# GATECH-EIC/BNS-GCN

Hardware: AMD Instinct MI355X
Metric: training throughput (full-graph edges/s), reddit-shaped graphsage 3-layer h=256, sampling-rate=0.1 (higher is better)
Workload: dtype fp32; 1 GPU; model=graphsage, dataset=reddit, n_layers=3, n_hidden=256, n_nodes=232965, n_edges=114756398, use_pp=True, partition=metis, parallelism=partition-parallel p1

## Files before the change

### bnsgcn_amd/ops/functional.py

```python
from __future__ import annotations

import torch
from torch.autograd import Function

from . import reference as ref
from ._ext import get_ext, use_hip



def _worklist_of(indptr):
    wl = getattr(indptr, "_bns_worklist", None)
    if wl is None:
        from .csr_torch import build_worklist
        wl = build_worklist(indptr)
        indptr._bns_worklist = wl
    return wl


def spmm_sum_raw(indptr, indices, x, src_scale=None, dst_scale=None, out=None):
    if use_hip(x):
        wrow, wbeg, wend, wave_start, zero_rows = _worklist_of(indptr)
        acc = out is not None
        if not acc:
            out = torch.empty(indptr.numel() - 1, x.shape[1],
# ... 180 lines not shown
                g_er = e.segment_sum_edges(*_worklist_of(indptr)[:4], None,
                                           grad, ctx.n_dst)
            return g_el, g_er, None, None, None, None, None, None
        if ctx.needs_input_grad[0]:
            g_el = torch.zeros(ctx.n_src, grad.shape[1], dtype=grad.dtype,
                               device=grad.device)
            g_el.index_add_(0, indices.long(), grad)
        if ctx.needs_input_grad[1]:
            g_er = torch.zeros(ctx.n_dst, grad.shape[1], dtype=grad.dtype,
                               device=grad.device)
            row = torch.repeat_interleave(
                torch.arange(ctx.n_dst, device=grad.device),
                indptr[1:] - indptr[:-1])
            g_er.index_add_(0, row, grad)
        return g_el, g_er, None, None, None, None, None, None


def sddmm_add(el, er, indptr, indices, indptr_t, indices_t, eperm_t,
              slope=None):
    return _SDDMMAdd.apply(el, er, indptr, indices, indptr_t, indices_t,
                           eperm_t, slope)


class _SegmentSoftmax(Function):
    @staticmethod
    def forward(ctx, logits, indptr):
        alpha = segment_softmax_raw(indptr, logits)
        ctx.save_for_backward(alpha, indptr)
        return alpha

    @staticmethod
    def backward(ctx, grad):
        alpha, indptr = ctx.saved_tensors
        return segment_softmax_bwd_raw(indptr, alpha, grad.contiguous()), None


def segment_softmax(logits, indptr):
    return _SegmentSoftmax.apply(logits, indptr)


import os as _os

_GEMM_MODE = _os.environ.get("BNSGCN_GEMM", "auto")


class _Linear(Function):

    @staticmethod
    def forward(ctx, x, weight, bias):
        ctx.save_for_backward(x, weight)
        ctx.has_bias = bias is not None
        if use_hip(x) and _GEMM_MODE == "hip":
            return get_ext().gemm_nt_bias(x, weight, bias)
        return torch.nn.functional.linear(x, weight, bias)

    @staticmethod
    def backward(ctx, grad):
        x, weight = ctx.saved_tensors
        grad = grad.contiguous()
        gx = gw = gb = None
        if use_hip(x):
            e = get_ext()
            if ctx.needs_input_grad[0]:
                gx = e.gemm_nn(grad, weight) if _GEMM_MODE == "hip" \
                    else grad @ weight
            if ctx.needs_input_grad[1]:
                gw = e.gemm_tn(grad, x)
            if ctx.has_bias and ctx.needs_input_grad[2]:
                return gx, gw, e.syncbn_stats(grad)[0]
        else:
            if ctx.needs_input_grad[0]:
                gx = grad @ weight
            if ctx.needs_input_grad[1]:
                gw = grad.t() @ x
        if ctx.has_bias and ctx.needs_input_grad[2]:
            gb = grad.sum(0)
        return gx, gw, gb


def linear(x, weight, bias=None):
    return _Linear.apply(x, weight, bias)


class _BiasAdd(Function):

    @staticmethod
    def forward(ctx, h, bias):
        return h + bias

    @staticmethod
    def backward(ctx, grad):
        gb = None
        if ctx.needs_input_grad[1]:
            gb = get_ext().syncbn_stats(grad.contiguous())[0] \
                if use_hip(grad) else grad.sum(0)
        return grad, gb


def bias_add(h, bias):
    return _BiasAdd.apply(h, bias)


class _LayerNormF(Function):

    @staticmethod
    def forward(ctx, x, weight, bias, eps, act):
        x = x.contiguous()
        y, mean, rstd = get_ext().ln_fwd(x, weight, bias, eps, int(act))
        ctx.save_for_backward(x, weight, bias, mean, rstd)
        ctx.act = int(act)
        return y

    @staticmethod
    def backward(ctx, dy):
        x, w, b, mean, rstd = ctx.saved_tensors
        dx, dw, db = get_ext().ln_bwd(x, dy.contiguous(), w, b, mean, rstd,
                                      ctx.act)
        return dx, dw, db, None, None


def layer_norm(x, weight, bias, eps: float = 1e-5, act: bool = False):
    if use_hip(x) and x.shape[-1] <= 1024 and x.dtype == torch.float32:
        return _LayerNormF.apply(x, weight, bias, eps, act)
    y = torch.nn.functional.layer_norm(x, (x.shape[-1],), weight, bias, eps)
    return torch.relu(y) if act else y


class _DropoutF(Function):

    @staticmethod
    def forward(ctx, x, keep, seed):
        ctx.keep, ctx.seed = keep, seed
        return get_ext().dropout_apply(x.contiguous(), keep, seed)

    @staticmethod
    def backward(ctx, dy):
        return (get_ext().dropout_apply(dy.contiguous(), ctx.keep, ctx.seed),
                None, None)


def dropout(x, p: float, training: bool):
    if not training or p <= 0.0:
        return x
    if use_hip(x) and x.dtype == torch.float32:
        seed = int(torch.randint(0, 2**62, (1,)).item())
        return _DropoutF.apply(x, 1.0 - p, seed)
    return torch.nn.functional.dropout(x, p, training)


def segment_softmax2_raw(indptr1, logits1, indptr2, logits2):
    if use_hip(logits1):
        return get_ext().segment_softmax2(indptr1, logits1, indptr2, logits2,
                                          1.0, 0)[:2]
    return ref.segment_softmax2(indptr1, logits1, indptr2, logits2)


def segment_softmax2_bwd_raw(indptr1, a1, g1, indptr2, a2, g2):
    if use_hip(a1):
        return get_ext().segment_softmax2_backward(indptr1, a1, g1,
                                                   indptr2, a2, g2, 1.0, 0)
    return ref.segment_softmax2_backward(indptr1, a1, g1, indptr2, a2, g2)


class _SegmentSoftmax2(Function):

    @staticmethod
# ... 67 lines not shown
```

### bnsgcn_amd/ops/hip/common.h

```cpp
#pragma once
#include <hip/hip_runtime.h>
#include <cstdint>

#define WAVE 64
#define DEV_INLINE __device__ __forceinline__

struct WorkList {
  const int32_t* __restrict__ row;
  const int64_t* __restrict__ beg;
  const int64_t* __restrict__ end;
  const int32_t* __restrict__ wave_start;
};

struct WaveItems { int lane, beg, end; };
struct WorkItem { int row; bool atomic; int64_t beg, end; };

DEV_INLINE int xcd_remap_block(int b, int nb) {
  const int q = nb / 8, r = nb % 8;
  const int xcd = b % 8, j = b / 8;
  return (xcd < r) ? xcd * (q + 1) + j : r * (q + 1) + (xcd - r) * q + j;
}

template <int SUBW>
DEV_INLINE WaveItems wave_items(const WorkList& wl) {
// ... 7 lines not shown
  const int row = wl.row[it];
  const bool atomic = row < 0;
  return {atomic ? ~row : row, atomic, wl.beg[it], wl.end[it]};
}

struct Chunk { int cid; float ssc; int nv; };

template <int SUBW>
DEV_INLINE Chunk load_chunk(const int32_t* __restrict__ indices,
                            const float* __restrict__ src_scale, int64_t e0,
                            int64_t end, int lane) {
  Chunk c = {0, 1.0f, (int)((end - e0 < SUBW) ? (end - e0) : SUBW)};
  if (lane < c.nv) {
    c.cid = indices[e0 + lane];
    if (src_scale) c.ssc = src_scale[c.cid];
  }
  return c;
}

DEV_INLINE void atomic_add(float* p, float v) { atomicAdd(p, v); }
DEV_INLINE void atomic_add(float2* p, float2 v) {
  float* f = reinterpret_cast<float*>(p);
  atomicAdd(f + 0, v.x); atomicAdd(f + 1, v.y);
}
DEV_INLINE void atomic_add(float4* p, float4 v) {
  float* f = reinterpret_cast<float*>(p);
  atomicAdd(f + 0, v.x); atomicAdd(f + 1, v.y);
  atomicAdd(f + 2, v.z); atomicAdd(f + 3, v.w);
}

template <bool ACC>
DEV_INLINE void store_row(float* dst, float v, bool atomic, float s = 1.0f) {
  if (atomic) atomic_add(dst, s * v);
  else if (ACC) *dst = fmaf(s, v, *dst);
  else *dst = s * v;
}
template <bool ACC>
DEV_INLINE void store_row(float2* dst, float2 v, bool atomic, float s = 1.0f) {
  if (atomic) {
    atomic_add(dst, make_float2(s * v.x, s * v.y));
  } else if (ACC) {
    const float2 pv = *dst;
    *dst = make_float2(fmaf(s, v.x, pv.x), fmaf(s, v.y, pv.y));
  } else {
    *dst = make_float2(s * v.x, s * v.y);
  }
}
template <bool ACC>
DEV_INLINE void store_row(float4* dst, float4 v, bool atomic, float s = 1.0f) {
  if (atomic) {
    atomic_add(dst, make_float4(s * v.x, s * v.y, s * v.z, s * v.w));
  } else if (ACC) {
    const float4 pv = *dst;
    *dst = make_float4(fmaf(s, v.x, pv.x), fmaf(s, v.y, pv.y),
                       fmaf(s, v.z, pv.z), fmaf(s, v.w, pv.w));
  } else {
    *dst = make_float4(s * v.x, s * v.y, s * v.z, s * v.w);
  }
}

DEV_INLINE uint32_t mulhi32(uint32_t a, uint32_t b) {
  return (uint32_t)(((uint64_t)a * b) >> 32);
}

struct P4 { uint32_t c0, c1, c2, c3; };

DEV_INLINE P4 philox4x32(uint32_t c0, uint32_t c1, uint32_t c2, uint32_t c3,
                         uint32_t k0, uint32_t k1) {
  const uint32_t M0 = 0xD2511F53u, M1 = 0xCD9E8D57u;
  const uint32_t W0 = 0x9E3779B9u, W1 = 0xBB67AE85u;
#pragma unroll
  for (int r = 0; r < 10; ++r) {
    uint32_t hi0 = mulhi32(c0, M0), lo0 = c0 * M0;
    uint32_t hi1 = mulhi32(c2, M1), lo1 = c2 * M1;
    uint32_t n0 = hi1 ^ c1 ^ k0;
    uint32_t n1 = lo1;
    uint32_t n2 = hi0 ^ c3 ^ k1;
    uint32_t n3 = lo0;
    c0 = n0; c1 = n1; c2 = n2; c3 = n3;
    k0 += W0; k1 += W1;
  }
  return {c0, c1, c2, c3};
}
```

### bnsgcn_amd/ops/hip/kernels.hip

```cpp
#include <hip/hip_runtime.h>
#include <torch/extension.h>
#include <ATen/cuda/CUDAContext.h>
#include <c10/util/Optional.h>
#include <algorithm>
#include "common.h"

namespace {


DEV_INLINE void f4_axpy(float4& a, float ss, const float4 v) {
  a.x += ss * v.x; a.y += ss * v.y; a.z += ss * v.z; a.w += ss * v.w;
}

template <bool ACC, int SUBW>
__global__ __launch_bounds__(256) void spmm_sum_vec4_kernel(
    const int32_t* __restrict__ wrow, const int64_t* __restrict__ wbeg,
    const int64_t* __restrict__ wend, const int32_t* __restrict__ wave_start,
    const int32_t* __restrict__ indices, const float* __restrict__ x,
    const float* __restrict__ src_scale, const float* __restrict__ dst_scale,
    float* __restrict__ out, int f4) {
  const WorkList wl = {wrow, wbeg, wend, wave_start};
  const WaveItems wi = wave_items<SUBW>(wl);
  const int lane = wi.lane;
  const float4* __restrict__ x4 = reinterpret_cast<const float4*>(x);
  float4* __restrict__ out4 = reinterpret_cast<float4*>(out);

  for (int it = wi.beg; it < wi.end; ++it) {
    const WorkItem wk = work_item(wl, it);
    const float ds = dst_scale ? dst_scale[wk.row] : 1.0f;
    for (int f0 = 0; f0 < f4; f0 += 2 * SUBW) {
      const int fA = f0 + lane;
      const int fB = fA + SUBW;
      const bool hasA = fA < f4, hasB = fB < f4;
      float4 acc0 = {0.f, 0.f, 0.f, 0.f}, acc1 = {0.f, 0.f, 0.f, 0.f};
      for (int64_t e0 = wk.beg; e0 < wk.end; e0 += SUBW) {
        const Chunk ch = load_chunk<SUBW>(indices, src_scale, e0, wk.end, lane);
#pragma unroll 4
        for (int k = 0; k < ch.nv; ++k) {
          const int c = __shfl(ch.cid, k, SUBW);
          const float ss = src_scale ? __shfl(ch.ssc, k, SUBW) : 1.0f;
          const int64_t base = (int64_t)c * f4;
          if (hasA) f4_axpy(acc0, ss, x4[base + fA]);
          if (hasB) f4_axpy(acc1, ss, x4[base + fB]);
        }
      }
      const int64_t ob = (int64_t)wk.row * f4;
      if (hasA) store_row<ACC>(&out4[ob + fA], acc0, wk.atomic, ds);
      if (hasB) store_row<ACC>(&out4[ob + fB], acc1, wk.atomic, ds);
    }
  }
}

template <bool ACC, int G>
__global__ __launch_bounds__(256) void spmm_sum_narrow_kernel(
    const int32_t* __restrict__ wrow, const int64_t* __restrict__ wbeg,
    const int64_t* __restrict__ wend, const int32_t* __restrict__ wave_start,
    const int32_t* __restrict__ indices, const float* __restrict__ x,
    const float* __restrict__ src_scale, const float* __restrict__ dst_scale,
    float* __restrict__ out, int f4) {
  constexpr int NG = WAVE / G;
  const WorkList wl = {wrow, wbeg, wend, wave_start};
  const WaveItems wi = wave_items<WAVE>(wl);
  const int lane = wi.lane;
  const int g = lane / G, j = lane % G;
  const bool has = j < f4;
  const float4* __restrict__ x4 = reinterpret_cast<const float4*>(x);
  float4* __restrict__ out4 = reinterpret_cast<float4*>(out);

  for (int it = wi.beg; it < wi.end; ++it) {
    const WorkItem wk = work_item(wl, it);
    const float ds = dst_scale ? dst_scale[wk.row] : 1.0f;
    float4 acc = {0.f, 0.f, 0.f, 0.f};
    for (int64_t e0 = wk.beg; e0 < wk.end; e0 += WAVE) {
      const Chunk ch = load_chunk<WAVE>(indices, src_scale, e0, wk.end, lane);
#pragma unroll 4
      for (int k = 0; k < ch.nv; k += NG) {
        const int kk = k + g;
        const int c = __shfl(ch.cid, kk, WAVE);
        const float ss = src_scale ? __shfl(ch.ssc, kk, WAVE) : 1.0f;
        if (has && kk < ch.nv) f4_axpy(acc, ss, x4[(int64_t)c * f4 + j]);
      }
    }
#pragma unroll
    for (int off = G; off < WAVE; off <<= 1) {
      acc.x += __shfl_xor(acc.x, off, WAVE);
      acc.y += __shfl_xor(acc.y, off, WAVE);
      acc.z += __shfl_xor(acc.z, off, WAVE);
      acc.w += __shfl_xor(acc.w, off, WAVE);
// ... 278 lines not shown
}


DEV_INLINE float wave_reduce_sum(float v) {
#pragma unroll
  for (int off = 32; off > 0; off >>= 1) v += __shfl_xor(v, off, WAVE);
  return v;
}

DEV_INLINE float wave_reduce_max(float v) {
#pragma unroll
  for (int off = 32; off > 0; off >>= 1) v = fmaxf(v, __shfl_xor(v, off, WAVE));
  return v;
}

__global__ __launch_bounds__(256) void sddmm_add_kernel(
    const int32_t* __restrict__ wrow, const int64_t* __restrict__ wbeg,
    const int64_t* __restrict__ wend, const int32_t* __restrict__ wave_start,
    const int32_t* __restrict__ indices, const float* __restrict__ el,
    const float* __restrict__ er, float* __restrict__ out, int H,
    float slope) {
  const WorkList wl = {wrow, wbeg, wend, wave_start};
  const WaveItems wi = wave_items<WAVE>(wl);
  for (int it = wi.beg; it < wi.end; ++it) {
    const WorkItem wk = work_item(wl, it);
    for (int64_t e0 = wk.beg; e0 < wk.end; e0 += WAVE) {
      const int64_t e = e0 + wi.lane;
      if (e >= wk.end) break;
      const int64_t c = indices[e];
      for (int h = 0; h < H; ++h) {
        float v = el[c * H + h] + er[(int64_t)wk.row * H + h];
        if (slope >= 0.f && v < 0.f) v *= slope;
        out[e * H + h] = v;
      }
    }
  }
}

__global__ void segment_softmax_kernel(const int64_t* __restrict__ indptr,
                                       const float* __restrict__ logits,
                                       float* __restrict__ alpha,
                                       int n_rows, int H) {
  const int wave = (blockIdx.x * blockDim.x + threadIdx.x) / WAVE;
  const int lane = threadIdx.x & (WAVE - 1);
  const int n_waves = (gridDim.x * blockDim.x) / WAVE;
  for (int rh = wave; rh < n_rows * H; rh += n_waves) {
    const int r = rh / H, h = rh % H;
    const int64_t beg = indptr[r], end = indptr[r + 1];
    if (beg == end) continue;
    float m = -INFINITY;
    for (int64_t e = beg + lane; e < end; e += WAVE)
      m = fmaxf(m, logits[e * H + h]);
    m = wave_reduce_max(m);
    float sum = 0.f;
    for (int64_t e = beg + lane; e < end; e += WAVE)
      sum += __expf(logits[e * H + h] - m);
    sum = wave_reduce_sum(sum);
    const float inv = 1.0f / fmaxf(sum, 1e-38f);
    for (int64_t e = beg + lane; e < end; e += WAVE)
      alpha[e * H + h] = __expf(logits[e * H + h] - m) * inv;
  }
}

__global__ void segment_softmax_bwd_kernel(const int64_t* __restrict__ indptr,
                                           const float* __restrict__ alpha,
                                           const float* __restrict__ grad,
                                           float* __restrict__ out,
                                           int n_rows, int H) {
  const int wave = (blockIdx.x * blockDim.x + threadIdx.x) / WAVE;
  const int lane = threadIdx.x & (WAVE - 1);
  const int n_waves = (gridDim.x * blockDim.x) / WAVE;
  for (int rh = wave; rh < n_rows * H; rh += n_waves) {
    const int r = rh / H, h = rh % H;
    const int64_t beg = indptr[r], end = indptr[r + 1];
    float sum = 0.f;
    for (int64_t e = beg + lane; e < end; e += WAVE)
      sum += alpha[e * H + h] * grad[e * H + h];
    sum = wave_reduce_sum(sum);
    for (int64_t e = beg + lane; e < end; e += WAVE)
      out[e * H + h] = alpha[e * H + h] * (grad[e * H + h] - sum);
  }
}

DEV_INLINE bool drop_keep(int64_t idx, uint32_t thr, uint64_t seed) {
  uint64_t z = seed + (uint64_t)idx;
  z = (z ^ (z >> 30)) * 0xBF58476D1CE4E5B9ull;
  z = (z ^ (z >> 27)) * 0x94D049BB133111EBull;
  z ^= z >> 31;
  return (uint32_t)(z >> 32) < thr;
}

DEV_INLINE uint32_t drop_threshold(float keep) {
  return (keep > 0.f && keep < 1.0f)
             ? (uint32_t)((double)keep * 4294967296.0) : 0u;
}

DEV_INLINE float drop_apply(float v, int64_t idx, uint32_t thr, uint64_t seed,
                            float inv_keep) {
  return drop_keep(idx, thr, seed) ? v * inv_keep : 0.f;
}

DEV_INLINE float4 drop_apply(float4 v, int64_t idx, uint32_t thr,
                             uint64_t seed, float inv_keep) {
  return make_float4(drop_apply(v.x, idx + 0, thr, seed, inv_keep),
                     drop_apply(v.y, idx + 1, thr, seed, inv_keep),
                     drop_apply(v.z, idx + 2, thr, seed, inv_keep),
                     drop_apply(v.w, idx + 3, thr, seed, inv_keep));
}

DEV_INLINE float4 f4_max(float4 a, float4 b) {
  return make_float4(fmaxf(a.x, b.x), fmaxf(a.y, b.y), fmaxf(a.z, b.z),
                     fmaxf(a.w, b.w));
}

DEV_INLINE float4 wave_reduce_sum4(float4 v) {
#pragma unroll
  for (int off = 32; off > 0; off >>= 1) {
    v.x += __shfl_xor(v.x, off, WAVE);
    v.y += __shfl_xor(v.y, off, WAVE);
    v.z += __shfl_xor(v.z, off, WAVE);
    v.w += __shfl_xor(v.w, off, WAVE);
  }
  return v;
}

DEV_INLINE float4 wave_reduce_max4(float4 v) {
#pragma unroll
  for (int off = 32; off > 0; off >>= 1) {
    float4 o = make_float4(__shfl_xor(v.x, off, WAVE),
                           __shfl_xor(v.y, off, WAVE),
                           __shfl_xor(v.z, off, WAVE),
                           __shfl_xor(v.w, off, WAVE));
    v = f4_max(v, o);
  }
  return v;
}


__global__ void segment_softmax2_h4_kernel(
    const int64_t* __restrict__ ip1, const float4* __restrict__ l1,
    const int64_t* __restrict__ ip2, const float4* __restrict__ l2,
    float4* __restrict__ a1, float4* __restrict__ a2,
    float4* __restrict__ da1, float4* __restrict__ da2,
    int n_rows, float keep, uint64_t seed, int64_t off2) {
  const int wave = (blockIdx.x * blockDim.x + threadIdx.x) / WAVE;
  const int lane = threadIdx.x & (WAVE - 1);
  const int n_waves = (gridDim.x * blockDim.x) / WAVE;
  const bool drop = keep < 1.0f;
  const uint32_t thr = drop_threshold(keep);
  const float inv_keep = drop ? 1.0f / keep : 1.0f;
  const int64_t* const ip[2] = {ip1, ip2};
  const float4* const l[2] = {l1, l2};
  float4* const a[2] = {a1, a2};
  float4* const da[2] = {da1, da2};
  const int64_t moff[2] = {0, off2};
  for (int r = wave; r < n_rows; r += n_waves) {
    const int64_t beg[2] = {ip[0][r], ip[1][r]};
    const int64_t end[2] = {ip[0][r + 1], ip[1][r + 1]};
    if (beg[0] == end[0] && beg[1] == end[1]) continue;
    float4 m = make_float4(-INFINITY, -INFINITY, -INFINITY, -INFINITY);
#pragma unroll
    for (int s = 0; s < 2; ++s)
      for (int64_t e = beg[s] + lane; e < end[s]; e += WAVE)
        m = f4_max(m, l[s][e]);
    m = wave_reduce_max4(m);
    float4 sum = make_float4(0.f, 0.f, 0.f, 0.f);
#pragma unroll
    for (int s = 0; s < 2; ++s)
      for (int64_t e = beg[s] + lane; e < end[s]; e += WAVE) {
        const float4 v = l[s][e];
        sum.x += __expf(v.x - m.x); sum.y += __expf(v.y - m.y);
        sum.z += __expf(v.z - m.z); sum.w += __expf(v.w - m.w);
      }
    sum = wave_reduce_sum4(sum);
    const float4 inv = make_float4(
        1.0f / fmaxf(sum.x, 1e-38f), 1.0f / fmaxf(sum.y, 1e-38f),
        1.0f / fmaxf(sum.z, 1e-38f), 1.0f / fmaxf(sum.w, 1e-38f));
#pragma unroll
    for (int s = 0; s < 2; ++s)
      for (int64_t e = beg[s] + lane; e < end[s]; e += WAVE) {
        const float4 v = l[s][e];
        float4 av;
        av.x = __expf(v.x - m.x) * inv.x; av.y = __expf(v.y - m.y) * inv.y;
        av.z = __expf(v.z - m.z) * inv.z; av.w = __expf(v.w - m.w) * inv.w;
        a[s][e] = av;
        if (drop)
          da[s][e] = drop_apply(av, moff[s] + e * 4, thr, seed, inv_keep);
      }
  }
}

// ... 1156 lines not shown
                                     at::Tensor ar) {
  check_f32(z, "z");
  const int64_t n = z.size(0);
  const int H = z.size(1), D = z.size(2);
  TORCH_CHECK(H <= 8 && (H * D) % 4 == 0, "attn_project shape limits");
  auto el = at::empty({n, H}, z.options());
  auto er = at::empty({n, H}, z.options());
  if (n == 0) return {el, er};
  auto stream = at::cuda::getCurrentCUDAStream();
  auto kfn = (D % 4 == 0) ? attn_project_fwd_kernel<true>
                          : attn_project_fwd_kernel<false>;
  hipLaunchKernelGGL(kfn, dim3(spmm_grid((int)std::min<int64_t>(n, 1 << 28))),
                     dim3(256), 0, stream, z.data_ptr<float>(),
                     al.data_ptr<float>(), ar.data_ptr<float>(),
                     el.data_ptr<float>(), er.data_ptr<float>(), n, H, D,
                     H * D / 4);
  return {el, er};
}

std::vector<at::Tensor> attn_project_backward(at::Tensor z, at::Tensor al,
                                              at::Tensor ar, at::Tensor g_el,
                                              at::Tensor g_er) {
  check_f32(z, "z");
  const int64_t n = z.size(0);
  const int H = z.size(1), D = z.size(2);
  const int HD = H * D;
  TORCH_CHECK(H <= 8 && HD % 4 == 0, "attn_project shape limits");
  auto dz = at::empty_like(z);
  auto dal = at::zeros({1, H, D}, z.options());
  auto dar = at::zeros({1, H, D}, z.options());
  if (n == 0) return {dz, dal, dar};
  auto stream = at::cuda::getCurrentCUDAStream();
  auto kfn = (D % 4 == 0) ? attn_project_dz_kernel<true>
                          : attn_project_dz_kernel<false>;
  hipLaunchKernelGGL(kfn,
                     dim3(spmm_grid((int)std::min<int64_t>(n, 1 << 28))),
                     dim3(256), 0, stream, al.data_ptr<float>(),
                     ar.data_ptr<float>(), g_el.data_ptr<float>(),
                     g_er.data_ptr<float>(), dz.data_ptr<float>(), n, H, D,
                     HD / 4);
  const int row_chunks = (int)std::min<int64_t>((n + 255) / 256, 2048);
  dim3 grid((HD + 255) / 256, row_chunks);
  hipLaunchKernelGGL(attn_project_dattn_kernel, grid, dim3(256), 0, stream,
                     z.data_ptr<float>(), g_el.data_ptr<float>(),
                     g_er.data_ptr<float>(), dal.data_ptr<float>(),
                     dar.data_ptr<float>(), n, H, D, HD, row_chunks);
  return {dz, dal, dar};
}

at::Tensor gemm_strided(const at::Tensor& A, int64_t sAm, int64_t sAk,
                        const at::Tensor& B, int64_t sBk, int64_t sBn,
                        const c10::optional<at::Tensor>& bias,
                        int M, int N, int K) {
  auto stream = at::cuda::getCurrentCUDAStream();
  if (M == 0 || N == 0) return at::zeros({M, N}, A.options());
  if (K == 0) {
    auto C = at::zeros({M, N}, A.options());
    if (bias.has_value()) C += *bias;
    return C;
  }
  dim3 grid((M + BM - 1) / BM, (N + BN - 1) / BN);
  const int base_blocks = grid.x * grid.y;
  int splitk = 1;
  if (base_blocks < 256 && K > 4 * BK) {
    splitk = std::min({(int)(768 / base_blocks), (K + 255) / 256, 64});
    splitk = std::max(splitk, 1);
  }
  if (splitk > 1) {
    auto C = at::zeros({M, N}, A.options());
    const int k_slice = ((K + splitk - 1) / splitk + BK - 1) / BK * BK;
    grid.z = (K + k_slice - 1) / k_slice;
    hipLaunchKernelGGL(gemm_f32_kernel<true>, grid, dim3(256), 0, stream,
                       A.data_ptr<float>(), sAm, sAk, B.data_ptr<float>(), sBk,
                       sBn, opt_ptr(bias), C.data_ptr<float>(), M, N, K, k_slice);
    return C;
  }
  auto C = at::empty({M, N}, A.options());
  hipLaunchKernelGGL(gemm_f32_kernel<false>, grid, dim3(256), 0, stream,
                     A.data_ptr<float>(), sAm, sAk, B.data_ptr<float>(), sBk,
                     sBn, opt_ptr(bias), C.data_ptr<float>(), M, N, K, K);
  return C;
}

at::Tensor gemm_nt_bias(at::Tensor x, at::Tensor w,
                        c10::optional<at::Tensor> bias) {
  check_f32(x, "x"); check_f32(w, "w");
  const int M = x.size(0), K = x.size(1), N = w.size(0);
  TORCH_CHECK(w.size(1) == K, "shape mismatch");
  return gemm_strided(x, K, 1, w, 1, K, bias, M, N, K);
}

at::Tensor gemm_nn(at::Tensor g, at::Tensor w) {
  check_f32(g, "g"); check_f32(w, "w");
  const int M = g.size(0), N = g.size(1), K = w.size(1);
  return gemm_strided(g, N, 1, w, K, 1, c10::nullopt, M, K, N);
}

at::Tensor gemm_tn(at::Tensor g, at::Tensor x) {
  check_f32(g, "g"); check_f32(x, "x");
  const int M = g.size(0), N = g.size(1), K = x.size(1);
  return gemm_strided(g, 1, N, x, K, 1, c10::nullopt, N, K, M);
}

}

PYBIND11_MODULE(TORCH_EXTENSION_NAME, m) {
  m.def("spmm_sum", &spmm_sum, "CSR SpMM sum with fused src/dst scales");
  m.def("pack_rows", &pack_rows, "gather rows + per-row scale");
  m.def("scatter_add_rows", &scatter_add_rows, "scatter-add rows + scale");
  m.def("philox_keys", &philox_keys, "BNS sampling keys (Philox4x32-10)");
  m.def("syncbn_stats", &syncbn_stats, "column sum + sum of squares");
  m.def("gemm_nt_bias", &gemm_nt_bias, "fp32 MFMA GEMM x@w^T+b");
  m.def("gemm_nn", &gemm_nn, "fp32 MFMA GEMM g@w");
  m.def("gemm_tn", &gemm_tn, "fp32 MFMA GEMM g^T@x");
  m.def("sddmm_add", &sddmm_add, "GAT u_add_v SDDMM");
  m.def("segment_softmax", &segment_softmax, "edge softmax by dst segment");
  m.def("segment_softmax_backward", &segment_softmax_backward,
        "edge softmax backward");
  m.def("segment_softmax2", &segment_softmax2,
        "union softmax over two edge sets (split GAT block)");
  m.def("segment_softmax2_backward", &segment_softmax2_backward,
        "union softmax backward");
  m.def("spmm_edge_sum", &spmm_edge_sum, "multi-head edge-weighted SpMM");
  m.def("sddmm_dot", &sddmm_dot, "per-edge per-head dot (spmm_edge grad)");
  m.def("bincount_i32", &bincount_i32, "atomic int32 histogram");
  m.def("ln_fwd", &ln_fwd, "row LayerNorm forward (y, mean, rstd); "
        "act=1 fuses ReLU");
  m.def("ln_bwd", &ln_bwd, "row LayerNorm backward (dx, dgamma, dbeta)");
  m.def("dropout_apply", &dropout_apply,
        "mask-free dropout (splitmix64; same kernel fwd and bwd)");
  m.def("attn_project", &attn_project, "fused GAT el/er projections");
  m.def("attn_project_backward", &attn_project_backward,
        "fused GAT projection backward");
  m.def("segment_sum_edges", &segment_sum_edges,
        "segment sum of (permuted) edge values by CSR row");
}
```

### setup.py

```python
import os
from setuptools import setup
from torch.utils.cpp_extension import BuildExtension, CUDAExtension

os.environ.setdefault("PYTORCH_ROCM_ARCH", "gfx950")

setup(
    name="bnsgcn_amd",
    version="0.1.0",
    ext_modules=[
        CUDAExtension(
            "bnsgcn_amd._C",
            sources=["bnsgcn_amd/ops/hip/kernels.hip"],
            depends=["bnsgcn_amd/ops/hip/common.h"],
            extra_compile_args={"nvcc": ["-O3"], "cxx": ["-O3"]},
        )
    ],
    cmdclass={"build_ext": BuildExtension},
)
```

Measured before the change: 3.967 billion edges/s.

## Add 128x128 MFMA tiled GEMM with auto-routing and fused dropout variants

Adds a new double-buffered 128x128x16 fp32 MFMA GEMM kernel with split-K for small tile counts, and routes gemm_nt/nn/tn to it by default when operands are aligned and padding waste is acceptable. It also adds dropout-fused GEMM entry points that apply a hash-based dropout mask while staging operands into LDS, so the dropped activation is never materialised. The intent is to raise GEMM efficiency through larger tiles and operand reuse, and to remove the separate dropout pass. The dropout_linear Python wrapper is defined but not wired into the model here, so only the tiled routing changes the default path; split-K uses atomics and a zeroed output.

```diff
diff --git a/bnsgcn_amd/ops/functional.py b/bnsgcn_amd/ops/functional.py
--- a/bnsgcn_amd/ops/functional.py
+++ b/bnsgcn_amd/ops/functional.py
@@ -286,6 +286,38 @@
     return _Linear.apply(x, weight, bias)
 
 
+class _DropoutLinear(Function):
+
+    @staticmethod
+    def forward(ctx, x, weight, bias, keep, seed):
+        x = x.contiguous()
+        ctx.save_for_backward(x, weight)
+        ctx.keep, ctx.seed = keep, seed
+        ctx.has_bias = bias is not None
+        return get_ext().gemm_nt_bias_drop(x, weight.contiguous(), bias,
+                                           keep, seed)
+
+    @staticmethod
+    def backward(ctx, grad):
+        x, weight = ctx.saved_tensors
+        grad = grad.contiguous()
+        e = get_ext()
+        gw = gb = None
+        if ctx.needs_input_grad[1]:
+            gw = e.gemm_tn_drop(grad, x, ctx.keep, ctx.seed)
+        if ctx.has_bias and ctx.needs_input_grad[2]:
+            gb = e.syncbn_stats(grad)[0]
+        return None, gw, gb, None, None
+
+
+def dropout_linear(x, weight, bias, p: float, training: bool):
+    if (training and p > 0.0 and use_hip(x) and x.dtype == torch.float32
+            and not x.requires_grad):
+        seed = int(torch.randint(0, 2**62, (1,)).item())
+        return _DropoutLinear.apply(x, weight, bias, 1.0 - p, seed)
+    return linear(dropout(x, p, training), weight, bias)
+
+
 class _BiasAdd(Function):
 
     @staticmethod
diff --git a/bnsgcn_amd/ops/hip/common.h b/bnsgcn_amd/ops/hip/common.h
--- a/bnsgcn_amd/ops/hip/common.h
+++ b/bnsgcn_amd/ops/hip/common.h
@@ -113,3 +113,29 @@
   }
   return {c0, c1, c2, c3};
 }
+
+DEV_INLINE bool drop_keep(int64_t idx, uint32_t thr, uint64_t seed) {
+  uint64_t z = seed + (uint64_t)idx;
+  z = (z ^ (z >> 30)) * 0xBF58476D1CE4E5B9ull;
+  z = (z ^ (z >> 27)) * 0x94D049BB133111EBull;
+  z ^= z >> 31;
+  return (uint32_t)(z >> 32) < thr;
+}
+
+DEV_INLINE uint32_t drop_threshold(float keep) {
+  return (keep > 0.f && keep < 1.0f)
+             ? (uint32_t)((double)keep * 4294967296.0) : 0u;
+}
+
+DEV_INLINE float drop_apply(float v, int64_t idx, uint32_t thr, uint64_t seed,
+                            float inv_keep) {
+  return drop_keep(idx, thr, seed) ? v * inv_keep : 0.f;
+}
+
+DEV_INLINE float4 drop_apply(float4 v, int64_t idx, uint32_t thr,
+                             uint64_t seed, float inv_keep) {
+  return make_float4(drop_apply(v.x, idx + 0, thr, seed, inv_keep),
+                     drop_apply(v.y, idx + 1, thr, seed, inv_keep),
+                     drop_apply(v.z, idx + 2, thr, seed, inv_keep),
+                     drop_apply(v.w, idx + 3, thr, seed, inv_keep));
+}
diff --git a/bnsgcn_amd/ops/hip/gemm_tiled.h b/bnsgcn_amd/ops/hip/gemm_tiled.h
--- /dev/null
+++ b/bnsgcn_amd/ops/hip/gemm_tiled.h
@@ -0,0 +1,21 @@
+#pragma once
+#include <ATen/ATen.h>
+#include <c10/util/Optional.h>
+#include <cstdint>
+
+namespace bns {
+
+enum GemmLayout { GEMM_NT = 0, GEMM_NN = 1, GEMM_TN = 2 };
+
+enum GemmDrop { DROP_NONE = 0, DROP_A = 1, DROP_B = 2 };
+
+bool gemm_tiled_aligned(GemmLayout layout, const at::Tensor& A,
+                        const at::Tensor& B, int M, int N, int R);
+
+at::Tensor gemm_tiled(GemmLayout layout, const at::Tensor& A,
+                      const at::Tensor& B,
+                      const c10::optional<at::Tensor>& bias, int M, int N,
+                      int R, GemmDrop drop = DROP_NONE, float keep = 1.0f,
+                      uint64_t seed = 0);
+
+}
diff --git a/bnsgcn_amd/ops/hip/gemm_tiled.hip b/bnsgcn_amd/ops/hip/gemm_tiled.hip
--- /dev/null
+++ b/bnsgcn_amd/ops/hip/gemm_tiled.hip
@@ -0,0 +1,294 @@
+#include <hip/hip_runtime.h>
+#include <ATen/cuda/CUDAContext.h>
+#include <c10/util/Exception.h>
+#include <algorithm>
+#include "common.h"
+#include "gemm_tiled.h"
+
+namespace {
+
+constexpr int TBM = 128, TBN = 128, TBK = 16;
+constexpr int KC_LD = TBK + 4;
+constexpr int KS_LD = 128;
+constexpr int KC_TILE = 128 * KC_LD;
+constexpr int KS_TILE = TBK * KS_LD;
+
+using f32x16 = __attribute__((ext_vector_type(16))) float;
+
+struct DropArgs { uint32_t thr; uint64_t seed; float inv_keep; };
+
+template <bool KC>
+DEV_INLINE void stage_coords(int tid, int j, int& row, int& k) {
+  if (KC) { row = (tid >> 2) + 64 * j; k = (tid & 3) * 4; }
+  else    { k = (tid >> 5) + 8 * j;    row = (tid & 31) * 4; }
+}
+
+template <bool KC, bool VEC>
+DEV_INLINE void stage_load(const float* __restrict__ P, int64_t ld, int r0,
+                           int R, int k0, int ke, int tid, float4 (&v)[2]) {
+#pragma unroll
+  for (int j = 0; j < 2; ++j) {
+    int row, k;
+    stage_coords<KC>(tid, j, row, k);
+    const int gr = r0 + row, gk = k0 + k;
+    const float* p = KC ? P + (int64_t)gr * ld + gk : P + (int64_t)gk * ld + gr;
+    float4 t = make_float4(0.f, 0.f, 0.f, 0.f);
+    if (VEC) {
+      if (gr < R && gk < ke) t = *reinterpret_cast<const float4*>(p);
+    } else {
+      const int lim = KC ? ((gr < R) ? ke - gk : 0) : ((gk < ke) ? R - gr : 0);
+      if (lim > 0) t.x = p[0];
+      if (lim > 1) t.y = p[1];
+      if (lim > 2) t.z = p[2];
+      if (lim > 3) t.w = p[3];
+    }
+    v[j] = t;
+  }
+}
+
+template <bool KC, bool DROP>
+DEV_INLINE void stage_store(float* __restrict__ S, int64_t ld, int r0, int k0,
+                            int tid, const float4 (&v)[2], const DropArgs& d) {
+#pragma unroll
+  for (int j = 0; j < 2; ++j) {
+    int row, k;
+    stage_coords<KC>(tid, j, row, k);
+    float4 t = v[j];
+    if (DROP) {
+      const int64_t idx = KC ? (int64_t)(r0 + row) * ld + (k0 + k)
+                             : (int64_t)(k0 + k) * ld + (r0 + row);
+      t = drop_apply(t, idx, d.thr, d.seed, d.inv_keep);
+    }
+    *reinterpret_cast<float4*>(S + (KC ? row * KC_LD + k : k * KS_LD + row)) = t;
+  }
+}
+
+template <bool KC>
+DEV_INLINE void frag_read(const float* __restrict__ S, int wo, int i, int h,
+                          int g, float (&o)[4][2]) {
+  if (KC) {
+#pragma unroll
+    for (int f = 0; f < 2; ++f) {
+      const float4 t = *reinterpret_cast<const float4*>(
+          S + (wo + f * 32 + i) * KC_LD + 8 * g + 4 * h);
+      o[0][f] = t.x; o[1][f] = t.y; o[2][f] = t.z; o[3][f] = t.w;
+    }
+  } else {
+#pragma unroll
+    for (int s = 0; s < 4; ++s) {
+      const float2 t = *reinterpret_cast<const float2*>(
+          S + (8 * g + 4 * h + s) * KS_LD + wo + 2 * i);
+      o[s][0] = t.x; o[s][1] = t.y;
+    }
+  }
+}
+
+template <bool KC>
+DEV_INLINE int frag_index(int f, int idx) {
+  return KC ? f * 32 + idx : 2 * idx + f;
+}
+
+template <bool A_KC, bool B_KC, bool VEC, int DROP, bool ATOMIC>
+__global__ __launch_bounds__(256)
+void gemm_tiled_kernel(const float* __restrict__ A, int64_t lda,
+                       const float* __restrict__ B, int64_t ldb,
+                       const float* __restrict__ bias, float* __restrict__ C,
+                       int M, int N, int K, int k_slice, int tiles_n,
+                       DropArgs drop) {
+  constexpr int A_TILE = A_KC ? KC_TILE : KS_TILE;
+  constexpr int B_TILE = B_KC ? KC_TILE : KS_TILE;
+  __shared__ __attribute__((aligned(16))) float lds[2 * (A_TILE + B_TILE)];
+
+  const int tid = threadIdx.x;
+  const int lane = tid & (WAVE - 1);
+  const int wid = tid / WAVE;
+  const int wr = (wid >> 1) * 64, wc = (wid & 1) * 64;
+  const int i_l = lane & 31, h_l = lane >> 5;
+  const int m0 = (blockIdx.x / tiles_n) * TBM;
+  const int n0 = (blockIdx.x % tiles_n) * TBN;
+  const int kb = blockIdx.y * k_slice;
+  const int ke = (kb + k_slice < K) ? kb + k_slice : K;
+
+  float4 ra[2], rb[2];
+  f32x16 acc[2][2];
+#pragma unroll
+  for (int fi = 0; fi < 2; ++fi)
+#pragma unroll
+    for (int fj = 0; fj < 2; ++fj)
+#pragma unroll
+      for (int r = 0; r < 16; ++r) acc[fi][fj][r] = 0.f;
+
+  stage_load<A_KC, VEC>(A, lda, m0, M, kb, ke, tid, ra);
+  stage_load<B_KC, VEC>(B, ldb, n0, N, kb, ke, tid, rb);
+  stage_store<A_KC, DROP == 1>(lds, lda, m0, kb, tid, ra, drop);
+  stage_store<B_KC, DROP == 2>(lds + A_TILE, ldb, n0, kb, tid, rb, drop);
+  __syncthreads();
+
+  int buf = 0;
+  for (int k0 = kb; k0 < ke; k0 += TBK) {
+    const bool more = (k0 + TBK) < ke;
+    if (more) {
+      stage_load<A_KC, VEC>(A, lda, m0, M, k0 + TBK, ke, tid, ra);
+      stage_load<B_KC, VEC>(B, ldb, n0, N, k0 + TBK, ke, tid, rb);
+    }
+    const float* As = lds + buf * (A_TILE + B_TILE);
+    const float* Bs = As + A_TILE;
+#pragma unroll
+    for (int g = 0; g < TBK / 8; ++g) {
+      float a[4][2], b[4][2];
+      frag_read<A_KC>(As, wr, i_l, h_l, g, a);
+      frag_read<B_KC>(Bs, wc, i_l, h_l, g, b);
+#pragma unroll
+      for (int s = 0; s < 4; ++s)
+#pragma unroll
+        for (int fi = 0; fi < 2; ++fi)
+#pragma unroll
+          for (int fj = 0; fj < 2; ++fj)
+            acc[fi][fj] = __builtin_amdgcn_mfma_f32_32x32x2f32(
+                a[s][fi], b[s][fj], acc[fi][fj], 0, 0, 0);
+    }
+    if (more) {
+      float* Wn = lds + (buf ^ 1) * (A_TILE + B_TILE);
+      stage_store<A_KC, DROP == 1>(Wn, lda, m0, k0 + TBK, tid, ra, drop);
+      stage_store<B_KC, DROP == 2>(Wn + A_TILE, ldb, n0, k0 + TBK, tid, rb,
+                                   drop);
+      __syncthreads();
+    }
+    buf ^= 1;
+  }
+
+  const bool add_bias = bias != nullptr && blockIdx.y == 0;
+#pragma unroll
+  for (int fi = 0; fi < 2; ++fi)
+#pragma unroll
+    for (int r = 0; r < 16; ++r) {
+      const int gm = m0 + wr +
+                     frag_index<A_KC>(fi, (r & 3) + 8 * (r >> 2) + 4 * h_l);
+      if (gm >= M) continue;
+      float* crow = C + (int64_t)gm * N;
+      if (!B_KC && VEC && !ATOMIC) {
+        const int gn = n0 + wc + 2 * i_l;
+        if (gn < N) {
+          float2 v = make_float2(acc[fi][0][r], acc[fi][1][r]);
+          if (add_bias) { v.x += bias[gn]; v.y += bias[gn + 1]; }
+          *reinterpret_cast<float2*>(crow + gn) = v;
+        }
+      } else {
+#pragma unroll
+        for (int fj = 0; fj < 2; ++fj) {
+          const int gn = n0 + wc + frag_index<B_KC>(fj, i_l);
+          if (gn < N) {
+            float v = acc[fi][fj][r];
+            if (add_bias) v += bias[gn];
+            if (ATOMIC) atomicAdd(crow + gn, v);
+            else crow[gn] = v;
+          }
+        }
+      }
+    }
+}
+
+struct LaunchArgs {
+  const float *A, *B, *bias;
+  float* C;
+  int64_t lda, ldb;
+  int M, N, K, k_slice, tiles_n;
+  dim3 grid;
+  DropArgs drop;
+  hipStream_t stream;
+};
+
+template <bool A_KC, bool B_KC, bool VEC, int DROP, bool ATOMIC>
+void launch_one(const LaunchArgs& a) {
+  hipLaunchKernelGGL((gemm_tiled_kernel<A_KC, B_KC, VEC, DROP, ATOMIC>),
+                     a.grid, dim3(256), 0, a.stream, a.A, a.lda, a.B, a.ldb,
+                     a.bias, a.C, a.M, a.N, a.K, a.k_slice, a.tiles_n, a.drop);
+}
+
+template <bool A_KC, bool B_KC, int DROP>
+void launch_layout(const LaunchArgs& a, bool vec, bool atomic) {
+  if (vec) {
+    if (atomic) launch_one<A_KC, B_KC, true, DROP, true>(a);
+    else        launch_one<A_KC, B_KC, true, DROP, false>(a);
+  } else {
+    if (atomic) launch_one<A_KC, B_KC, false, DROP, true>(a);
+    else        launch_one<A_KC, B_KC, false, DROP, false>(a);
+  }
+}
+
+inline bool aligned16(const at::Tensor& t) {
+  return reinterpret_cast<uintptr_t>(t.data_ptr<float>()) % 16 == 0;
+}
+
+}
+
+namespace bns {
+
+bool gemm_tiled_aligned(GemmLayout layout, const at::Tensor& A,
+                        const at::Tensor& B, int M, int N, int R) {
+  if (!aligned16(A) || !aligned16(B)) return false;
+  switch (layout) {
+    case GEMM_NT: return R % 4 == 0;
+    case GEMM_NN: return R % 4 == 0 && N % 4 == 0;
+    default:      return M % 4 == 0 && N % 4 == 0;
+  }
+}
+
+at::Tensor gemm_tiled(GemmLayout layout, const at::Tensor& A,
+                      const at::Tensor& B,
+                      const c10::optional<at::Tensor>& bias, int M, int N,
+                      int R, GemmDrop drop, float keep, uint64_t seed) {
+  TORCH_CHECK(M > 0 && N > 0 && R > 0, "gemm_tiled: empty operand");
+  LaunchArgs a;
+  a.A = A.data_ptr<float>();
+  a.B = B.data_ptr<float>();
+  a.bias = bias.has_value() ? bias->data_ptr<float>() : nullptr;
+  a.lda = (layout == GEMM_TN) ? M : R;
+  a.ldb = (layout == GEMM_NT) ? R : N;
+  a.M = M; a.N = N; a.K = R;
+  a.stream = at::cuda::getCurrentCUDAStream();
+  const bool vec = gemm_tiled_aligned(layout, A, B, M, N, R);
+
+  const bool dropping = drop != DROP_NONE && keep < 1.0f;
+  a.drop.thr = (keep > 0.f && keep < 1.0f)
+                   ? (uint32_t)((double)keep * 4294967296.0) : 0u;
+  a.drop.seed = seed;
+  a.drop.inv_keep = dropping ? 1.0f / keep : 1.0f;
+
+  const int tiles_m = (M + TBM - 1) / TBM;
+  a.tiles_n = (N + TBN - 1) / TBN;
+  const int64_t tiles = (int64_t)tiles_m * a.tiles_n;
+  constexpr int64_t kResidentBlocks = 512;
+  int splitk = 1;
+  if (tiles < kResidentBlocks && R >= 16 * TBK) {
+    splitk = (int)std::min<int64_t>(kResidentBlocks / tiles,
+                                    (int64_t)R / (8 * TBK));
+    splitk = std::max(splitk, 1);
+  }
+  a.k_slice = R;
+  if (splitk > 1) {
+    a.k_slice = ((R + splitk - 1) / splitk + TBK - 1) / TBK * TBK;
+    splitk = (R + a.k_slice - 1) / a.k_slice;
+  }
+  const bool atomic = splitk > 1;
+  a.grid = dim3((unsigned)tiles, (unsigned)splitk);
+  auto C = atomic ? at::zeros({M, N}, A.options())
+                  : at::empty({M, N}, A.options());
+  a.C = C.data_ptr<float>();
+
+  if (layout == GEMM_NT) {
+    TORCH_CHECK(drop != DROP_B, "gemm_tiled: NT drops A");
+    if (dropping) launch_layout<true, true, 1>(a, vec, atomic);
+    else          launch_layout<true, true, 0>(a, vec, atomic);
+  } else if (layout == GEMM_NN) {
+    TORCH_CHECK(drop == DROP_NONE, "gemm_tiled: NN has no dropout form");
+    launch_layout<true, false, 0>(a, vec, atomic);
+  } else {
+    TORCH_CHECK(drop != DROP_A, "gemm_tiled: TN drops B");
+    if (dropping) launch_layout<false, false, 2>(a, vec, atomic);
+    else          launch_layout<false, false, 0>(a, vec, atomic);
+  }
+  return C;
+}
+
+}
diff --git a/bnsgcn_amd/ops/hip/kernels.hip b/bnsgcn_amd/ops/hip/kernels.hip
--- a/bnsgcn_amd/ops/hip/kernels.hip
+++ b/bnsgcn_amd/ops/hip/kernels.hip
@@ -4,6 +4,7 @@
 #include <c10/util/Optional.h>
 #include <algorithm>
 #include "common.h"
+#include "gemm_tiled.h"
 
 namespace {
 
@@ -448,31 +449,6 @@
   }
 }
 
-DEV_INLINE bool drop_keep(int64_t idx, uint32_t thr, uint64_t seed) {
-  uint64_t z = seed + (uint64_t)idx;
-  z = (z ^ (z >> 30)) * 0xBF58476D1CE4E5B9ull;
-  z = (z ^ (z >> 27)) * 0x94D049BB133111EBull;
-  z ^= z >> 31;
-  return (uint32_t)(z >> 32) < thr;
-}
-
-DEV_INLINE uint32_t drop_threshold(float keep) {
-  return (keep > 0.f && keep < 1.0f)
-             ? (uint32_t)((double)keep * 4294967296.0) : 0u;
-}
-
-DEV_INLINE float drop_apply(float v, int64_t idx, uint32_t thr, uint64_t seed,
-                            float inv_keep) {
-  return drop_keep(idx, thr, seed) ? v * inv_keep : 0.f;
-}
-
-DEV_INLINE float4 drop_apply(float4 v, int64_t idx, uint32_t thr,
-                             uint64_t seed, float inv_keep) {
-  return make_float4(drop_apply(v.x, idx + 0, thr, seed, inv_keep),
-                     drop_apply(v.y, idx + 1, thr, seed, inv_keep),
-                     drop_apply(v.z, idx + 2, thr, seed, inv_keep),
-                     drop_apply(v.w, idx + 3, thr, seed, inv_keep));
-}
 
 DEV_INLINE float4 f4_max(float4 a, float4 b) {
   return make_float4(fmaxf(a.x, b.x), fmaxf(a.y, b.y), fmaxf(a.z, b.z),
@@ -1795,24 +1771,67 @@
   return C;
 }
 
+enum { GEMM_AUTO = 0, GEMM_OLD = 1, GEMM_TILED = 2 };
+
+bool route_tiled(bns::GemmLayout layout, const at::Tensor& A,
+                 const at::Tensor& B, int M, int N, int R, int64_t kernel) {
+  TORCH_CHECK(kernel >= GEMM_AUTO && kernel <= GEMM_TILED, "bad kernel id");
+  if (kernel == GEMM_OLD || M == 0 || N == 0 || R == 0) return false;
+  if (kernel == GEMM_TILED) return true;
+  if (!bns::gemm_tiled_aligned(layout, A, B, M, N, R) || R < 32) return false;
+  auto pad = [](int64_t v, int64_t t) { return (v + t - 1) / t * t; };
+  return 4 * pad(M, 128) * pad(N, 128) <= 5 * pad(M, BM) * pad(N, BN);
+}
+
 at::Tensor gemm_nt_bias(at::Tensor x, at::Tensor w,
-                        c10::optional<at::Tensor> bias) {
+                        c10::optional<at::Tensor> bias, int64_t kernel) {
   check_f32(x, "x"); check_f32(w, "w");
   const int M = x.size(0), K = x.size(1), N = w.size(0);
   TORCH_CHECK(w.size(1) == K, "shape mismatch");
+  if (route_tiled(bns::GEMM_NT, x, w, M, N, K, kernel))
+    return bns::gemm_tiled(bns::GEMM_NT, x, w, bias, M, N, K);
   return gemm_strided(x, K, 1, w, 1, K, bias, M, N, K);
 }
 
-at::Tensor gemm_nn(at::Tensor g, at::Tensor w) {
+at::Tensor gemm_nn(at::Tensor g, at::Tensor w, int64_t kernel) {
   check_f32(g, "g"); check_f32(w, "w");
   const int M = g.size(0), N = g.size(1), K = w.size(1);
+  TORCH_CHECK(w.size(0) == N, "shape mismatch");
+  if (route_tiled(bns::GEMM_NN, g, w, M, K, N, kernel))
+    return bns::gemm_tiled(bns::GEMM_NN, g, w, c10::nullopt, M, K, N);
   return gemm_strided(g, N, 1, w, K, 1, c10::nullopt, M, K, N);
 }
 
-at::Tensor gemm_tn(at::Tensor g, at::Tensor x) {
+at::Tensor gemm_tn(at::Tensor g, at::Tensor x, int64_t kernel) {
   check_f32(g, "g"); check_f32(x, "x");
   const int M = g.size(0), N = g.size(1), K = x.size(1);
+  TORCH_CHECK(x.size(0) == M, "shape mismatch");
+  if (route_tiled(bns::GEMM_TN, g, x, N, K, M, kernel))
+    return bns::gemm_tiled(bns::GEMM_TN, g, x, c10::nullopt, N, K, M);
   return gemm_strided(g, 1, N, x, K, 1, c10::nullopt, N, K, M);
+}
+
+at::Tensor gemm_nt_bias_drop(at::Tensor x, at::Tensor w,
+                             c10::optional<at::Tensor> bias, double keep,
+                             int64_t seed) {
+  check_f32(x, "x"); check_f32(w, "w");
+  const int M = x.size(0), K = x.size(1), N = w.size(0);
+  TORCH_CHECK(w.size(1) == K, "shape mismatch");
+  if (M == 0 || N == 0 || K == 0)
+    return gemm_strided(x, K, 1, w, 1, K, bias, M, N, K);
+  return bns::gemm_tiled(bns::GEMM_NT, x, w, bias, M, N, K, bns::DROP_A,
+                         (float)keep, (uint64_t)seed);
+}
+
+at::Tensor gemm_tn_drop(at::Tensor g, at::Tensor x, double keep,
+                        int64_t seed) {
+  check_f32(g, "g"); check_f32(x, "x");
+  const int M = g.size(0), N = g.size(1), K = x.size(1);
+  TORCH_CHECK(x.size(0) == M, "shape mismatch");
+  if (M == 0 || N == 0 || K == 0)
+    return gemm_strided(g, 1, N, x, K, 1, c10::nullopt, N, K, M);
+  return bns::gemm_tiled(bns::GEMM_TN, g, x, c10::nullopt, N, K, M,
+                         bns::DROP_B, (float)keep, (uint64_t)seed);
 }
 
 }
@@ -1823,9 +1842,16 @@
   m.def("scatter_add_rows", &scatter_add_rows, "scatter-add rows + scale");
   m.def("philox_keys", &philox_keys, "BNS sampling keys (Philox4x32-10)");
   m.def("syncbn_stats", &syncbn_stats, "column sum + sum of squares");
-  m.def("gemm_nt_bias", &gemm_nt_bias, "fp32 MFMA GEMM x@w^T+b");
-  m.def("gemm_nn", &gemm_nn, "fp32 MFMA GEMM g@w");
-  m.def("gemm_tn", &gemm_tn, "fp32 MFMA GEMM g^T@x");
+  m.def("gemm_nt_bias", &gemm_nt_bias, "fp32 MFMA GEMM x@w^T+b",
+        py::arg("x"), py::arg("w"), py::arg("bias"), py::arg("kernel") = 0);
+  m.def("gemm_nn", &gemm_nn, "fp32 MFMA GEMM g@w", py::arg("g"),
+        py::arg("w"), py::arg("kernel") = 0);
+  m.def("gemm_tn", &gemm_tn, "fp32 MFMA GEMM g^T@x", py::arg("g"),
+        py::arg("x"), py::arg("kernel") = 0);
+  m.def("gemm_nt_bias_drop", &gemm_nt_bias_drop,
+        "tiled GEMM dropout(x)@w^T+b, dropout fused into the operand load");
+  m.def("gemm_tn_drop", &gemm_tn_drop,
+        "tiled GEMM g^T@dropout(x), dropout fused into the operand load");
   m.def("sddmm_add", &sddmm_add, "GAT u_add_v SDDMM");
   m.def("segment_softmax", &segment_softmax, "edge softmax by dst segment");
   m.def("segment_softmax_backward", &segment_softmax_backward,
diff --git a/setup.py b/setup.py
--- a/setup.py
+++ b/setup.py
@@ -10,8 +10,10 @@
     ext_modules=[
         CUDAExtension(
             "bnsgcn_amd._C",
-            sources=["bnsgcn_amd/ops/hip/kernels.hip"],
-            depends=["bnsgcn_amd/ops/hip/common.h"],
+            sources=["bnsgcn_amd/ops/hip/kernels.hip",
+                     "bnsgcn_amd/ops/hip/gemm_tiled.hip"],
+            depends=["bnsgcn_amd/ops/hip/common.h",
+                     "bnsgcn_amd/ops/hip/gemm_tiled.h"],
             extra_compile_args={"nvcc": ["-O3"], "cxx": ["-O3"]},
         )
     ],
```

New measurement: 4.097 billion edges/s, median of 6. +3.3%, better.
